# robotic-vision-lab/Learning-Implicitly-From-Spatial-Transformers-Network

Measured on AMD Instinct MI355X. Metric: SDF query-points/sec (B=8, N=20k, 224^2), higher is better.
Workload: dtype fp16

## Files before the change

learning-implicitly-from-spatial-transformers-network_amd/csrc/fused_fc0_kernels.hip:

```cpp
#include "list_common.h"
#include "mfma_common.h"
#include "point_math.h"
#include "gather_math.h"

namespace list {

constexpr int kFusedLds = 163840;
constexpr int kFW = 65536, kFA = 16384;
constexpr int kFAOff = 2 * kFW;


__device__ __forceinline__ int fswz(int row) { return (row >> 1) & 7; }

struct RowProj { int64_t base; int dx, dy; float w00, w01, w10, w11; int valid; };
struct RowProjRec { int64_t base; int dx, dy; float w00, w01, w10, w11; int valid, pad_[3]; };
constexpr int kFProjRecOff = 81920;

template <int X3, bool PROJ = false>
__global__ __launch_bounds__(512, 2) void k_fc0_fused(FusedFc0Params fp) {
  static_assert(!PROJ || X3 == 0, "the projected form is built for fp16 operands");
  constexpr bool F16 = X3 == 0;
  constexpr int KT = F16 ? 64 : 32;
  using M = MapT<F16 ? 1 : 0>;
  __shared__ __attribute__((aligned(16))) char smem[kFusedLds];
  const GemmParams& p = fp.gp;
  const int tid = threadIdx.x;
  const int lane = tid & 63;
  const int wave = __builtin_amdgcn_readfirstlane(tid >> 6);
  const int wm = wave >> 2, wn = wave & 3;
  const int ntiles = p.M / 128;
  const int m0 = xcd_contiguous_block(blockIdx.x, ntiles) * 128;
  const int nk = p.K / KT;
  const int np = fp.n_produced;
  const int64_t lda = (int64_t)(p.lda ? p.lda : p.K) * (F16 ? 2 : 4), ldw = lda;
  const int gap_at = p.k_gap_at, gap = p.k_gap;
  auto ktb = [&](int t) { return (t + (t >= gap_at ? gap : 0)) * 128; };

  const int pc = tid & 7, pr = tid >> 3;
  RowProj rp[2];
  if (np > 0 || PROJ) {
#pragma unroll
    for (int h = 0; h < 2; ++h) {
      const Pt pt = load_point(fp.g, m0 + pr + 64 * h);
      const Proj q = project(fp.trans_mat + pt.b * 12, pt.x, pt.y, pt.z, fp.ms, fp.Ct, fp.clamp_hi);
      rp[h].base = (int64_t)pt.b * fp.ms * fp.ms * fp.Ct + q.o00 + pc * M::V;
      rp[h].dx = q.o01 - q.o00; rp[h].dy = q.o10 - q.o00;
      rp[h].w00 = q.w00; rp[h].w01 = q.w01; rp[h].w10 = q.w10; rp[h].w11 = q.w11;
      rp[h].valid = (pt.valid ? 1 : 0) | (q.dead << 1);
    }
  }
  typename M::Raw taps[2][4];
  auto load_taps = [&](int t) {
#pragma unroll
    for (int h = 0; h < 2; ++h) {
      const int64_t o = rp[h].base + t * KT;
      taps[h][0] = M::load(fp.img_map, o);
      taps[h][1] = M::load(fp.img_map, o + rp[h].dx);
      taps[h][2] = M::load(fp.img_map, o + rp[h].dy);
      taps[h][3] = M::load(fp.img_map, o + rp[h].dy + rp[h].dx);
    }
  };
  auto produce = [&](char* astage) {
#pragma unroll
// ... 120 lines not shown
    if (t + 1 < np) {
      wait_vmcnt<8>();
      produce(smem + kFAOff + nxt * kFA);
      if (t + 2 < np) load_taps(t + 2);
    }
  }

  {
    float* tile = (float*)smem + wave * (32 * kStageLd);
    const int col_in = lane & 15, row_in = 4 * (lane >> 4);
    const int rr = lane >> 3, c8 = (lane & 7) * 8;
    const int64_t row_base = m0 + wm * 64;
    const int col_base = wn * 128;
    bool bad = false;
    __syncthreads();
    const RowProjRec* recs = (const RowProjRec*)(smem + kFProjRecOff);
    if constexpr (PROJ) {
      if (pc == 0) {
#pragma unroll
        for (int h = 0; h < 2; ++h) {
          RowProjRec rc;
          rc.base = rp[h].base; rc.dx = rp[h].dx; rc.dy = rp[h].dy;
          rc.w00 = rp[h].w00; rc.w01 = rp[h].w01; rc.w10 = rp[h].w10; rc.w11 = rp[h].w11; rc.valid = rp[h].valid;
          rc.pad_[0] = rc.pad_[1] = rc.pad_[2] = 0;
          *(RowProjRec*)(smem + kFProjRecOff + (pr + 64 * h) * (int)sizeof(RowProjRec)) = rc;
        }
      }
      __syncthreads();
    }
#pragma unroll
    for (int ih = 0; ih < 2; ++ih)
#pragma unroll
      for (int jh = 0; jh < 2; ++jh) {
        [[maybe_unused]] uint4 ptap[4][4];
        if constexpr (PROJ) {
#pragma unroll
          for (int k = 0; k < 4; ++k) {
            const RowProjRec& rc = recs[wm * 64 + ih * 32 + rr + 8 * k];
            const int64_t o = rc.base + fp.kept + col_base + jh * 64 + c8;
            ptap[k][0] = M::load(fp.img_map, o);
            ptap[k][1] = M::load(fp.img_map, o + rc.dx);
            ptap[k][2] = M::load(fp.img_map, o + rc.dy);
            ptap[k][3] = M::load(fp.img_map, o + rc.dy + rc.dx);
          }
        }
#pragma unroll
        for (int ii = 0; ii < 2; ++ii)
#pragma unroll
          for (int jj = 0; jj < 4; ++jj)
#pragma unroll
            for (int e = 0; e < 4; ++e)
              tile[(ii * 16 + row_in + e) * kStageLd + jj * 16 + col_in] = acc[2 * ih + ii][4 * jh + jj][e];
        __syncthreads();
        const int cb = col_base + jh * 64 + c8;
        const float4 b0 = *(const float4*)(p.bias + cb), b1 = *(const float4*)(p.bias + cb + 4);
        const float bb[8] = {b0.x, b0.y, b0.z, b0.w, b1.x, b1.y, b1.z, b1.w};
#pragma unroll
        for (int k = 0; k < 4; ++k) {
          const int r = rr + 8 * k;
          const float4 x = *(const float4*)(tile + r * kStageLd + c8);
          const float4 y = *(const float4*)(tile + r * kStageLd + c8 + 4);
          const float v[8] = {x.x, x.y, x.z, x.w, y.x, y.y, y.z, y.w};
          float o[8];
          if constexpr (PROJ) {
            const RowProjRec& rc = recs[wm * 64 + ih * 32 + r];
            const float wt[4] = {rc.w00, rc.w01, rc.w10, rc.w11};
            float sm[8];
#pragma unroll
            for (int e = 0; e < 8; ++e) sm[e] = 0.f;
#pragma unroll
            for (int tp = 0; tp < 4; ++tp) {
              float f[8];
              M::unpack(ptap[k][tp], f);
              const bool dead = (rc.valid >> (1 + tp)) & 1;
#pragma unroll
              for (int e = 0; e < 8; ++e) sm[e] = fmaf(dead ? 0.f : f[e], wt[tp], sm[e]);
            }
            const bool live = (rc.valid & 1) != 0;
#pragma unroll
            for (int e = 0; e < 8; ++e) { o[e] = relu_nan((v[e] + (live ? sm[e] : 0.f)) + bb[e]); bad = bad || (o[e] != o[e]); }
          } else {
#pragma unroll
            for (int e = 0; e < 8; ++e) { o[e] = relu_nan(v[e] + bb[e]); bad = bad || (o[e] != o[e]); }
          }
          store8_planes<F16 ? 1 : 0>(p.out_hi, F16 ? nullptr : p.out_lo, (row_base + ih * 32 + r) * p.ldo + cb, o);
        }
        __syncthreads();
      }
    if (p.nan_tiles && __builtin_amdgcn_ballot_w64(bad) != 0 && lane == 0) p.nan_tiles[m0 / 256] = 1;
  }
}

bool fused_fc0_eligible(const GemmParams& gp, int img_f16, int img_C) {
  if (gp.N != 512 || gp.M <= 0 || gp.M % 128 || gp.K % 64 || img_C < 0 || img_C % 64 || img_C > gp.K || !gp.bias ||
      gp.rowvec || gp.a_rows || gp.tile_gate) return false;
  if (gp.lda != gp.ldw || (gp.k_gap && !gp.lda)) return false;
  return gp.fmt == FMT_FP16 ? (img_f16 != 0 && !gp.x3i) : (img_f16 == 0 && gp.x3i != 0);
}

hipError_t launch_fc0_fused(const FusedFc0Params& fp, int terms, hipStream_t s) {
  const dim3 grid(fp.gp.M / 128);
  if (fp.proj) {
    if (fp.gp.fmt != FMT_FP16 || fp.gp.N != 512) return hipErrorInvalidValue;
    hipLaunchKernelGGL((k_fc0_fused<0, true>), grid, dim3(512), 0, s, fp);
  } else if (fp.gp.fmt == FMT_FP16) hipLaunchKernelGGL((k_fc0_fused<0, false>), grid, dim3(512), 0, s, fp);
  else if (terms == 3) hipLaunchKernelGGL((k_fc0_fused<3, false>), grid, dim3(512), 0, s, fp);
  else hipLaunchKernelGGL((k_fc0_fused<1, false>), grid, dim3(512), 0, s, fp);
  return hipGetLastError();
}

}
```

learning-implicitly-from-spatial-transformers-network_amd/csrc/gather_kernels.hip:

```cpp
#include <string.h>

#include "list_common.h"
#include "point_math.h"
#include "gather_math.h"

namespace list {

template <int V>
__device__ __forceinline__ bool any_nan(const float (&a)[V]) {
  bool bad = false;
#pragma unroll
  for (int c = 0; c < V; ++c) bad = bad || (a[c] != a[c]);
  return bad;
}
__device__ __forceinline__ bool wave_any(bool x) { return __builtin_amdgcn_ballot_w64(x) != 0; }
__device__ __forceinline__ void launder(float& x) { asm volatile("" : "+v"(x)); }
__device__ __forceinline__ void launder(int& x) { asm volatile("" : "+v"(x)); }
__device__ __forceinline__ void launder(unsigned& x) { asm volatile("" : "+v"(x)); }
__device__ __forceinline__ void launder(float4& r) { launder(r.x); launder(r.y); launder(r.z); launder(r.w); }
__device__ __forceinline__ void launder(uint4& r) { launder(r.x); launder(r.y); launder(r.z); launder(r.w); }

template <typename M>
__device__ __forceinline__ void tap_fma_masked(typename M::Raw r, float w, bool dead, float (&a)[M::V]) {
  float f[M::V];
// ... 460 lines not shown
      p.z = q[(int64_t)g.perm2 * g.q_sc] * g.scale;
      if (p.valid) row = g.row_of[pt];
    } else {
      p = load_point(g, row);
    }
    ImgPoint ip;
    ip.pr = project(trans_mat + p.b * 12, p.x, p.y, p.z, ms, Ct, clamp_hi);
    ip.row = row; ip.b = p.b; ip.valid = p.valid ? 1 : 0;
    ipt[threadIdx.x] = ip;
  }
  __syncthreads();
  unsigned short* __restrict__ xh = g.x_hi;
  unsigned short* __restrict__ xl = g.x_lo;
  const int64_t img_stride = (int64_t)ms * ms * Ct;
  constexpr int NP = 2;
  const int lq = Ct / M::V;
  const int ppp = lq >= 256 ? 1 : 256 / lq;
  const int span = ppp * NP;
#pragma unroll 1
  for (int i = 0; i < kGatherRows; i += span) {
    for (int u = threadIdx.x; u < ppp * lq; u += 256) {
      const int pp = u / lq, q = u - pp * lq;
      Raw v[NP][4];
#pragma unroll
      for (int k = 0; k < NP; ++k) {
        const int pi = min(i + k * ppp + pp, kGatherRows - 1);
        const ImgPoint& a = ipt[pi];
        const int64_t bo = a.b * img_stride + q * M::V;
        v[k][0] = M::load(img_map, bo + a.pr.o00); v[k][1] = M::load(img_map, bo + a.pr.o01);
        v[k][2] = M::load(img_map, bo + a.pr.o10); v[k][3] = M::load(img_map, bo + a.pr.o11);
      }
// ... 4 lines not shown
        const ImgPoint& a = ipt[pi];
        float r[M::V];
        if constexpr (OUT32) {
          if (q * M::V >= kept) {
            reduce_proj_exact<M>(v[k], a.pr, r);
            float* dst = g.rowvec + (int64_t)a.row * g.rv_stride + (q * M::V - kept);
#pragma unroll
            for (int h = 0; h < M::V / 4; ++h)
              *(float4*)(dst + 4 * h) = a.valid ? make_float4(r[4 * h], r[4 * h + 1], r[4 * h + 2], r[4 * h + 3])
                                                : make_float4(0.f, 0.f, 0.f, 0.f);
            continue;
          }
        }
        tap_mul<M>(v[k][0], a.pr.w00, r); tap_fma<M>(v[k][1], a.pr.w01, r);
        tap_fma<M>(v[k][2], a.pr.w10, r); tap_fma<M>(v[k][3], a.pr.w11, r);
        store_feats<FMT, M::V, true>(xh, xl, (int64_t)a.row * g.Kp + col_off + q * M::V, r, a.valid != 0);
      }
    }
  }
}

template <int FMT>
__global__ __launch_bounds__(256) void k_copy_percep(GatherParams g, const float* __restrict__ pf,
                                                     int64_t sb, int64_t sc, int64_t sn, int Ct,
                                                     int col_off) {
  const int row = blockIdx.x * 256 + threadIdx.x;
  if (row >= g.rows) return;
  const bool valid = row < g.n_valid;
  const int64_t gp = g.p_begin + (valid ? (g.order ? g.order[row] : row) : 0);
  const int b = (int)(gp / g.N);
  const int n = (int)(gp - (int64_t)b * g.N);
// ... 241 lines not shown
      case 64: return launch_vox_level<64, FMT>(g, lv, L.vox_off[l], s, order, rd);
      case 128: return launch_vox_level<128, FMT>(g, lv, L.vox_off[l], s, order, rd);
      case 256: return launch_vox_level<256, FMT>(g, lv, L.vox_off[l], s, order, rd);
      default: return hipErrorInvalidValue;
    }
  };
  auto img = [&]() -> hipError_t {
    if (skip_img) return hipSuccess;
    if (a.percep_proj) {
      if (FMT == FMT_FP16)
        LIST_LAUNCH((k_gather_img<FMT, 1, 1>), dim3(g.rows / kGatherRows), dim3(256), 0, s, order, g, a.percep_proj,
                    a.trans_mat, a.map_size, a.H1, a.clamp_hi, 0, 0);
      else
        LIST_LAUNCH((k_gather_img<FMT, 0, 1>), dim3(g.rows / kGatherRows), dim3(256), 0, s, order, g, a.percep_proj,
                    a.trans_mat, a.map_size, a.H1, a.clamp_hi, 0, 0);
    } else if (a.img_proj) {
      if (FMT == FMT_FP16)
        LIST_LAUNCH((k_gather_img<FMT, 1, 1>), dim3(g.rows / kGatherRows), dim3(256), 0, s, order, g, a.img_map,
                    a.trans_mat, a.map_size, a.img_kept_C + a.H1, a.clamp_hi, L.img_off, a.img_kept_C);
      else
        LIST_LAUNCH((k_gather_img<FMT, 0, 1>), dim3(g.rows / kGatherRows), dim3(256), 0, s, order, g, a.img_map,
                    a.trans_mat, a.map_size, a.img_kept_C + a.H1, a.clamp_hi, L.img_off, a.img_kept_C);
    } else if (a.percep_feat) {
      LIST_LAUNCH(k_copy_percep<FMT>, dim3((g.rows + 255) / 256), dim3(256), 0, s, order, g,
                  a.percep_feat, a.pf_sb, a.pf_sc, a.pf_sn, L.img_C, L.img_off);
    } else if (a.img_dtype == LIST_MAP_F16) {
      LIST_LAUNCH((k_gather_img<FMT, 1>), dim3(g.rows / kGatherRows), dim3(256), 0, s, order, g, a.img_map,
                  a.trans_mat, a.map_size, L.img_C, a.clamp_hi, L.img_off, 0);
    } else {
      LIST_LAUNCH((k_gather_img<FMT, 0>), dim3(g.rows / kGatherRows), dim3(256), 0, s, order, g, a.img_map,
// ... 116 lines not shown
```

learning-implicitly-from-spatial-transformers-network_amd/csrc/gemm_kernels.hip:

```cpp
#include <type_traits>

#include "list_common.h"
#include "mfma_common.h"

namespace list {

constexpr int BM = 256, BN = 256;
constexpr int kLdsBytes = 131072;

template <int TERMS> struct Pipe {
  static constexpr int kPlanes = TERMS == 3 ? 4 : 2;
  static constexpr int BK = TERMS == 3 ? 32 : 64;
  static constexpr int kRowBytes = BK * 2;
  static constexpr int kPlaneBytes = BM * kRowBytes;
  static constexpr int kStageBytes = kPlanes * kPlaneBytes;
  static constexpr int kStages = kLdsBytes / kStageBytes;
  static constexpr int kAhead = kStages - 1;
  static constexpr int kRowsPerPiece = 1024 / kRowBytes;
  static constexpr int kPiecesPerWave = BM / kRowsPerPiece / 8;
  static constexpr int kLoadsPerStage = kPiecesPerWave * kPlanes;
  static constexpr int kWOff = (TERMS == 3 ? 2 : 1) * kPlaneBytes;
  __device__ static __forceinline__ int swz(int row) {
    return kRowBytes == 64 ? ((row >> 2) & 3) : ((row >> 1) & 7);
  }
// ... 339 lines not shown
          store8_planes<FP16>(p.out_hi, p.out_lo, (row_base + c * 32 + r) * p.ldo + col_base + c8, o);
        }
        __syncthreads();
      }
    } else
    staged_epilogue16(acc, smem, wave, lane, [&](int r, int c8, const float (&v)[8]) {
      float o[8];
      const float4 b0 = p.bias ? *(const float4*)(p.bias + col_base + c8) : make_float4(0.f, 0.f, 0.f, 0.f);
      const float4 b1 = p.bias ? *(const float4*)(p.bias + col_base + c8 + 4) : make_float4(0.f, 0.f, 0.f, 0.f);
      const float bb[8] = {b0.x, b0.y, b0.z, b0.w, b1.x, b1.y, b1.z, b1.w};
#pragma unroll
      for (int e = 0; e < 8; ++e) { o[e] = relu_nan(v[e] + bb[e]); bad = bad || (o[e] != o[e]); }
      store8_planes<FP16>(p.out_hi, p.out_lo, (row_base + r) * p.ldo + col_base + c8, o);
    });
    if (p.nan_tiles && __builtin_amdgcn_ballot_w64(bad) != 0 && lane == 0) p.nan_tiles[m0 / BM] = 1;
  } else if (EPI == EPI_MASK_SPLIT) {
    const int64_t row_base = m0 + wm * 128;
    const int col_base = n0 + wn * 64;
    staged_epilogue16(acc, smem, wave, lane, [&](int r, int c8, const float (&v)[8]) {
      const int64_t row = row_base + r;
      const uint4 mk = *(const uint4*)(p.mask + row * p.ldmask + col_base + c8);
      const unsigned mw[4] = {mk.x, mk.y, mk.z, mk.w};
      float o[8];
#pragma unroll
      for (int e = 0; e < 4; ++e) {
        o[2 * e] = (mw[e] & 0x7fffu) ? v[2 * e] : 0.f;
        o[2 * e + 1] = (mw[e] & 0x7fff0000u) ? v[2 * e + 1] : 0.f;
      }
      store8_planes<FP16>(p.out_hi, p.out_lo, row * p.ldo + col_base + c8, o);
    });
// ... 84 lines not shown
    }
  }
}

__device__ __forceinline__ int a_quarter_row(int q, int half) { return (q >> 3) * 128 + half * 64 + (q & 7) * 8; }
__device__ __forceinline__ int w_quarter_row(int q, int half) { return (q >> 2) * 64 + half * 32 + (q & 3) * 8; }

constexpr int kLead = 4;
constexpr int kPpMinK = 512;

template <int EPI, int FP16, bool S16, int X3 = 0>
__global__ __launch_bounds__(512, 2) void k_gemm_nt_pp(GemmParams p) {
  using P = Pipe<1>;
  static_assert(X3 == 0 || (S16 && !FP16), "interleaved split operands: 16x16x32 bf16 only");
  static_assert(P::BK == 64 && P::kRowBytes == 128, "single-plane pipeline");
  __shared__ __attribute__((aligned(16))) char smem[kLdsBytes];
  const int lane = threadIdx.x & 63;
  const int wave = __builtin_amdgcn_readfirstlane(threadIdx.x >> 6);
  const int wm = wave >> 2, wn = wave & 3;
  const int tiles_n = p.N / BN;
  const int ntiles = (p.M / BM) * tiles_n;
  const int tile = xcd_contiguous_block(blockIdx.x, ntiles);
  int m0 = (tile / tiles_n) * BM;
  const int n0 = (tile % tiles_n) * BN;
  if (p.tile_gate && p.tile_gate[tile / tiles_n] == 0) return;
  const char* A = p.a_hi; const char* Wt = p.w_hi;
  int Kk = p.K, lda_e = p.lda ? p.lda : p.K, a_rows_e = p.a_rows ? p.a_rows : p.M;
  [[maybe_unused]] void* dx_out = p.dx;
  if constexpr (EPI == EPI_DX) {
    if (p.n_groups > 0) {
      int mt = tile / tiles_n;
// ... 33 lines not shown
  const int w_row_off = (wn * 64 + frow) * P::kRowBytes;
  const int64_t lda = (int64_t)lda_e * (X3 ? 4 : 2);
  const int64_t ldw = (int64_t)(p.ldw ? p.ldw : p.K) * (X3 ? 4 : 2);
  const int a_last = a_rows_e - 1;
  const int nk = X3 ? Kk / 32 : Kk / P::BK;

  auto stage_quarter = [&](char* sbase, int kbyte, int quarter) {
#pragma unroll
    for (int r = 0; r < 2; ++r) {
      const int q = 2 * wave + r;
      const bool is_a = quarter == 0 || quarter == 3;
      const int row0 = is_a ? a_quarter_row(q, quarter == 3) : w_quarter_row(q, quarter == 2);
      const int row = row0 + lane / 8;
      const int chunk = (lane % 8) ^ P::swz(row);
      const char* g = (is_a ? A + (int64_t)min(m0 + row, a_last) * lda : Wt + (int64_t)(n0 + row) * ldw) + kbyte + chunk * 16;
      if (EPI == EPI_RELU_SPLIT && is_a) glds16_nt(g, sbase + row0 * P::kRowBytes);
      else glds16(g, sbase + (is_a ? 0 : P::kWOff) + row0 * P::kRowBytes);
    }
  };
  auto frag = [&](const char* cur, int plane_off, int row_off, int blk, int ks) -> bf16x8 {
    return *(const bf16x8*)(cur + plane_off + row_off + blk * TR * P::kRowBytes + (((KO * ks + fo) ^ fswz) << 4));
  };

  const int gap_at = p.k_gap_at, gap = p.k_gap;
  auto ktb = [&](int t) { return (t + (t >= gap_at ? gap : 0)) * P::kRowBytes; };
#pragma unroll
  for (int g = 0; g < kLead; ++g)
    if (g / 4 < nk) stage_quarter(smem + ((g / 4) & 1) * P::kStageBytes, ktb(g / 4), g & 3);
  if (nk > 1) wait_vmcnt<2 * (kLead - 4)>(); else wait_vmcnt<0>();
  __builtin_amdgcn_s_barrier();
  if (wm == 1) __builtin_amdgcn_s_barrier();
  const int last_quarter = 4 * nk - 1;

  bf16x8 a[HA][KS], w[2][HW][KS];
  auto k_tile = [&](int t, auto steady) {
    constexpr bool STEADY = decltype(steady)::value;
    const char* cur = smem + (t & 1) * P::kStageBytes;
#pragma unroll
    for (int ph = 0; ph < 4; ++ph) {
      if (ph == 0 || ph == 1) {
#pragma unroll
        for (int ks = 0; ks < KS; ++ks)
#pragma unroll
// ... 314 lines not shown
    hipLaunchKernelGGL((k_gemm_nt<TERMS, EPI, FP16>), dim3(ntiles), dim3(512), 0, s, p);
  }
  return hipGetLastError();
}

template <int TERMS, int FP16>
static hipError_t launch_epi(const GemmParams& p, int epi, hipStream_t s) {
  if (epi == EPI_RELU_SPLIT) return launch_one<TERMS, EPI_RELU_SPLIT, FP16>(p, s);
  if (epi == EPI_F32) return launch_one<TERMS, EPI_F32, FP16>(p, s);
  if (epi == EPI_MASK_SPLIT) return launch_one<TERMS, EPI_MASK_SPLIT, FP16>(p, s);
  if (epi == EPI_DX) return launch_one<TERMS, EPI_DX, FP16>(p, s);
  return launch_one<TERMS, EPI_RELU_DOT, FP16>(p, s);
}

hipError_t launch_gemm(const GemmParams& p, int terms, int epi, hipStream_t s) {
  if (p.n_groups) {
    if (epi != EPI_DX || p.n_groups < 0 || p.n_groups > kGemmMaxGroups) return hipErrorInvalidValue;
    int tiles = 0;
    for (int i = 0; i < p.n_groups; ++i) {
      const GemmGroup& g = p.grp[i];
      if (g.K % 64 || g.K <= 0 || g.m_tiles <= 0 || g.a_rows <= 0 || g.a_rows > g.m_tiles * BM || !g.a || !g.w || !g.out) return hipErrorInvalidValue;
      tiles += g.m_tiles;
    }
    if (tiles * BM != p.M || p.plain_loop) return hipErrorInvalidValue;
  }
  if (p.M % BM || p.N % BN || p.K % 64 || p.M <= 0) return hipErrorInvalidValue;
  if (p.x3i && p.fmt == FMT_FP16) return hipErrorInvalidValue;
  if (epi == EPI_RELU_DOT && p.N != BN) return hipErrorInvalidValue;
  if (p.fmt == FMT_FP16) return launch_epi<1, 1>(p, epi, s);
  if (terms == 3) return launch_epi<3, 0>(p, epi, s);
// ... 5 lines not shown
```

learning-implicitly-from-spatial-transformers-network_amd/csrc/list_capi.hip:

```cpp
#include <string.h>

#include "list_common.h"
#include "list_host.h"

using namespace list;

namespace {

constexpr int64_t kMaxChunkRows = 262144;

bool aligned16(const void* p) { return (reinterpret_cast<uintptr_t>(p) & 15) == 0; }

bool vox_in_place(const ListMap3D& m, ListVoxLevel* lv, int32_t map_dtype) {
  const int64_t C = m.C, W = m.W, H = m.H;
  lv->C = m.C; lv->D = m.D; lv->H = m.H; lv->W = m.W; lv->dtype = LIST_MAP_F32; lv->reserved_ = 0;
  if (m.dtype == LIST_MAP_F16) {
    if (map_dtype != LIST_MAP_F16 || m.C == 1 || (m.C % 8) != 0) return false;
    if (m.sc == 1 && m.sw == C && m.sh == W * C && m.sd == H * W * C && aligned16(m.data) && (m.sb % 8) == 0) {
      lv->data = m.data; lv->image_stride = m.sb; lv->dtype = LIST_MAP_F16; return true;
    }
    return false;
  }
  if (m.C == 1) {
    if (m.sw == 1 && m.sh == W && m.sd == H * W) { lv->data = m.data; lv->image_stride = m.sb; return true; }
// ... 109 lines not shown
  while (fit >= kRowTile && workspace_layout(fit, Kp, H1, H2).total > bytes) fit -= kRowTile;
  return fit >= kRowTile ? fit : 0;
}

int fused_fc0_mode() {
  static const int mode = [] {
    const char* e = getenv("LIST_FUSED_FC0");
    if (!e || !e[0]) return 1;
    if (e[0] == '0' && e[1] == 0) return 0;
    if (e[0] == 'x') return 2;
    if (e[0] == '3' && e[1] == 0) return 3;
    return 1;
  }();
  return mode;
}
bool takes_fused_fc0_any(const ListQueryArgs* a, const FeatLayout& L) {
  if (fused_fc0_mode() == 0) return false;
  if (a->percep_feat || a->percep_proj) return false;
  if (a->img_proj && (a->precision != LIST_PREC_FP16 || fused_fc0_mode() == 2)) return false;
  if ((a->precision == LIST_PREC_FP16) != (a->img_dtype == LIST_MAP_F16)) return false;
  if (a->precision == LIST_PREC_BF16X3 && fused_fc0_mode() != 3) return false;
  if (!a->no_activations || a->no_fused_fc0) return false;
  return a->H1 == 512 && a->img_C > 0 && a->img_C % 64 == 0 && L.img_off == 0 && L.Kp % 64 == 0;
}
int fused_produced_tiles(const ListQueryArgs* a) {
  const int channels = a->img_proj ? a->img_kept_C : a->img_C;
  return fused_fc0_mode() == 2 ? 0 : channels / (a->precision == LIST_PREC_FP16 ? 64 : 32);
}
bool takes_fused_fc0(const ListQueryArgs* a, const FeatLayout& L) {
  return takes_fused_fc0_any(a, L) && fused_fc0_mode() != 2;
}

bool takes_fused_tail(const ListQueryArgs* a) {
  return a->no_activations && a->precision == LIST_PREC_FP16 && a->H2 == 256 && a->H3 == 256 && a->H1 % 64 == 0;
}

}

extern "C" {

const char* list_last_error(void) { return g_err; }
int list_abi_version(void) { return LIST_ABI_VERSION; }

static bool dtype_ok(int32_t d) { return d == LIST_MAP_F32 || d == LIST_MAP_F16; }
static size_t elem_bytes(int32_t d) { return d == LIST_MAP_F16 ? 2 : 4; }
// ... 364 lines not shown
  const int sets = a->stage_events ? (a->stage_event_sets > 0 ? a->stage_event_sets : 1) : 0;
  int chunk = 0;
  for (int64_t p0 = 0; p0 < P; p0 += rows, ++chunk) {
    const int n_valid = (int)((P - p0 < rows) ? (P - p0) : rows);
    const int crow = (n_valid + kRowTile - 1) / kRowTile * kRowTile;
    GatherParams g = make_gather(a, L, ws, p0, n_valid, crow);
    void* const* events = chunk < sets ? a->stage_events + (size_t)chunk * LIST_N_STAGES : nullptr;
    chunk_args.stage_events = events;
    auto mark = [&](int stage) {
      if (events && events[stage]) (void)hipEventRecord((hipEvent_t)events[stage], s);
    };
    mark(LIST_STAGE_BEGIN);
    hipError_t e = hipSuccess;
    if (!a->no_sort) {
      SortBuffers sb;
      const bool want_pix = !takes_fused_fc0(a, L);
      sb.order = (int*)(wsb + ws.order); sb.order_img = want_pix ? (int*)(wsb + ws.order_img) : nullptr;
      sb.row_of = (int*)(wsb + ws.row_of); sb.keys = (int*)(wsb + ws.keys);
      sb.keys2 = (int*)(wsb + ws.keys2); sb.bins = (int*)(wsb + ws.bins);
      e = launch_sort_points(g, *a, sb, s);
      if (e != hipSuccess) return hip_fail(e, "sort launch");
      g.order = sb.order;
      if (want_pix && a->percep_feat == nullptr && a->map_size * ((a->map_size + 3) / 4) <= kSortPixCells) {
        g.order_img = sb.order_img; g.row_of = sb.row_of;
      }
    }
    mark(LIST_STAGE_SORT);
    int* nan_tiles = (int*)(wsb + ws.nan_tiles);
    const bool fused0 = takes_fused_fc0_any(a, L);
    e = launch_gather(g, L, chunk_args, nan_tiles, s, takes_fused_fc0(a, L));
    if (e != hipSuccess) return hip_fail(e, "gather launch");
    mark(LIST_STAGE_TAIL);

    GemmParams gp;
    memset(&gp, 0, sizeof(gp));
    gp.fmt = g.fmt;
    gp.a_hi = wsb + ws.x_hi; gp.a_lo = wsb + ws.x_lo;
    gp.w_hi = wp + pk.w0_hi; gp.w_lo = wp + pk.w0_lo;
    gp.bias = (const float*)(wp + pk.b0);
    gp.M = crow; gp.N = a->H1; gp.K = L.Kp;
    gp.x3i = g.fmt == FMT_FP16 ? 0 : 1;
    if (gp.x3i && (ws.x_lo != ws.x_hi + (size_t)rows * L.Kp * 2 || pk.w0_lo != pk.w0_hi + (size_t)a->H1 * L.Kp * 2))
      return fail(LIST_ERR_ARG, "internal: hi / lo planes of X or of the packed fc_0 weight are not contiguous");
    if (a->percep_proj) {
      const int64_t skip = (int64_t)a->img_C * (gp.x3i ? 4 : 2);
// ... 4 lines not shown
      const int ktile = gp.x3i ? 32 : 64;
      gp.k_gap_at = a->img_kept_C / ktile; gp.k_gap = (a->img_C - a->img_kept_C) / ktile;
      gp.K = L.Kp - (a->img_C - a->img_kept_C); gp.lda = L.Kp; gp.ldw = L.Kp;
      gp.rowvec = (const char*)g.rowvec; gp.rowvec_stride = g.rv_stride * 4;
      if (a->H1 * 4 > L.Kp * 2) return fail(LIST_ERR_UNSUPPORTED, "img_proj: H1 * 4 bytes exceed a row of the feature matrix's lo plane");
    }
    const char* rowvec_of_call = gp.rowvec;
    gp.out_hi = (unsigned short*)(wsb + ws.h1_hi);
    gp.out_lo = terms == 3 ? (unsigned short*)(wsb + ws.h1_lo) : nullptr;
    gp.ldo = a->H1;
    gp.nan_tiles = nan_tiles;
    if (fused0) {
      FusedFc0Params fp;
      fp.gp = gp; fp.g = g; fp.img_map = a->img_map; fp.trans_mat = a->trans_mat;
      fp.ms = a->map_size; fp.Ct = a->img_C; fp.clamp_hi = a->clamp_hi; fp.n_produced = fused_produced_tiles(a);
      fp.proj = 0; fp.kept = 0;
      if (a->img_proj) {
        fp.proj = 1; fp.kept = a->img_kept_C; fp.Ct = a->img_kept_C + a->H1; fp.gp.rowvec = nullptr;
      }
      if (!fused_fc0_eligible(fp.gp, a->img_dtype == LIST_MAP_F16, a->img_proj ? a->img_kept_C : a->img_C))
        return fail(LIST_ERR_ARG, "internal: fused fc_0 taken for arguments it does not support");
      e = launch_fc0_fused(fp, terms, s);
    } else {
      e = launch_gemm(gp, terms, EPI_RELU_SPLIT, s);
    }
    if (e != hipSuccess) return hip_fail(e, "fc_0 launch");
    mark(LIST_STAGE_FC0);
    e = launch_gather_fixup(g, L, chunk_args, nan_tiles, s);
    if (e != hipSuccess) return hip_fail(e, "gather fix-up launch");
    gp.nan_tiles = nullptr; gp.tile_gate = nan_tiles; gp.rowvec = rowvec_of_call;
    e = launch_gemm(gp, terms, EPI_RELU_SPLIT, s);
    if (e != hipSuccess) return hip_fail(e, "gated fc_0 launch");
    gp.tile_gate = nullptr; gp.x3i = 0;
    gp.lda = gp.ldw = 0; gp.rowvec = nullptr; gp.k_gap_at = gp.k_gap = 0;
    mark(LIST_STAGE_EXACT);
    gp.a_hi = wsb + ws.h1_hi; gp.a_lo = wsb + ws.h1_lo;
    gp.w_hi = wp + pk.w1_hi; gp.w_lo = wp + pk.w1_lo;
// ... 39 lines not shown
  if (a->H1 <= 0 || a->H2 <= 0) return fail(LIST_ERR_UNSUPPORTED, "hidden sizes %d/%d/%d", a->H1, a->H2, a->H3);
  const int64_t P = (int64_t)a->B * a->N;
  const int64_t rows = chunk_rows_for(a->workspace_bytes, P, L.Kp, a->H1, a->H2);
  if (rows < kRowTile) return fail(LIST_ERR_WORKSPACE, "workspace of %zu bytes cannot hold one %d-row tile",
                                   a->workspace_bytes, kRowTile);
  plan->rows_per_chunk = rows;
  plan->chunks = (int32_t)((P + rows - 1) / rows);
  plan->fused_tail = takes_fused_tail(a) ? 1 : 0;
  plan->fc0_k = a->percep_proj ? L.Kp - a->img_C : a->img_proj ? L.Kp - (a->img_C - a->img_kept_C) : L.Kp;
  plan->img_proj = a->img_proj ? 1 : 0;
  {
    const Workspace ws = workspace_layout(rows, L.Kp, a->H1, a->H2);
    const int n_valid = (int)(P < rows ? P : rows);
    const GatherParams g = make_gather(a, L, ws, 0, n_valid, (n_valid + kRowTile - 1) / kRowTile * kRowTile);
    plan->box_levels = gather_box_levels(g, L, *a);
    plan->fused_fc0 = takes_fused_fc0(a, L) ? 1 : 0;
  }
  return LIST_OK;
}

int list_gather_features_fwd(const ListQueryArgs* a, float* out, void* stream) {
  FeatLayout L;
  int rc = check_query_common(a, &L);
  if (rc != LIST_OK) return rc;
  if (!out) return fail(LIST_ERR_ARG, "out is NULL");
  if (a->percep_proj || a->img_proj) return fail(LIST_ERR_UNSUPPORTED, "percep_proj / img_proj leave perceptual features out of X");
  const int64_t P = (int64_t)a->B * a->N;
  const int H1 = a->H1 > 0 ? a->H1 : 512, H2 = a->H2 > 0 ? a->H2 : 256;
  const int64_t rows = chunk_rows_for(a->workspace_bytes, P, L.Kp, H1, H2);
  if (rows < kRowTile) return fail(LIST_ERR_WORKSPACE, "workspace too small");
  const Workspace ws = workspace_layout(rows, L.Kp, H1, H2);
// ... 475 lines not shown
```

learning-implicitly-from-spatial-transformers-network_amd/csrc/list_common.h:

```cpp
#pragma once

#include <hip/hip_runtime.h>
#include <hip/hip_ext.h>
#include <stdint.h>
#include <stdlib.h>

#include "list_hip.h"

namespace list {

inline int any_order() {
  static const int flag = [] {
    const char* e = getenv("LIST_LAUNCH_IN_ORDER");
    return (e && e[0] && !(e[0] == '0' && e[1] == 0)) ? 0 : (int)hipExtAnyOrderLaunch;
  }();
  return flag;
}
#define LIST_LAUNCH(kernel, grid, block, lds, s, order, ...) \
  hipExtLaunchKernelGGL(kernel, grid, block, lds, s, nullptr, nullptr, (order), __VA_ARGS__)

template <bool FP16, typename V>
__device__ __forceinline__ void x_store(const V& v, V* p) {
  if (FP16) *p = v;
  else __builtin_nontemporal_store(v, p);
// ... 303 lines not shown
  float* out_f32; int relu;
  const float* w3; const float* b3; float* sdf; int n_valid;
  const int* order;
  int fmt;
  const unsigned short* mask; int ldmask;
  void* dx; int dx_f16; int n_store;
  int plain_loop;
  int* nan_tiles;
  const int* tile_gate;
  int x3i;
  int lda, ldw;
  int a_rows;
  const char* rowvec; int64_t rowvec_stride;
  GemmGroup grp[kGemmMaxGroups]; int n_groups;
  int k_gap_at, k_gap;
};

enum { EPI_RELU_SPLIT = 0, EPI_F32 = 1, EPI_RELU_DOT = 2, EPI_MASK_SPLIT = 3, EPI_DX = 4 };

struct GemmTnParams {
  const char* a_hi; const char* a_lo; int lda;
  const char* b_hi; const char* b_lo; int ldb;
  int M, N, P;
  int splits, steps_per_split;
  float* slab; int ldn;
  int fmt;
  int b_x3i;
};

hipError_t launch_prep_img(const ListMap2D maps[LIST_N_IMG_LEVELS], int B, int map_size, int Ct,
                           int f16, void* out, hipStream_t s, int n_levels = LIST_N_IMG_LEVELS);
hipError_t launch_img_level_rows(const ListMap2D* maps, void* const* outs, int n, int B, int f16, hipStream_t s);
hipError_t launch_proj_resize_sum(const ListMap2D* src, int n_src, int B, int map_size, int Ct, int coff, int f16,
// ... 16 lines not shown
                               hipStream_t s);
bool gather_box_eligible(const GatherParams& g, const ListVoxLevel& lv, int col_off);
hipError_t launch_gather_vox_box(const GatherParams& g, const ListVoxLevel& lv, int col_off, hipStream_t s, int order);
int gather_box_levels(const GatherParams& g, const FeatLayout& L, const ListQueryArgs& a);
hipError_t launch_gather_fixup(const GatherParams& g, const FeatLayout& L, const ListQueryArgs& a,
                               const int* tile_flags, hipStream_t s);
hipError_t launch_percep_pool(const ListPoolArgs& a, hipStream_t s);
hipError_t launch_gemm(const GemmParams& p, int terms, int epi, hipStream_t s);
struct FusedFc0Params {
  GemmParams gp;
  GatherParams g;
  const void* img_map;
  const float* trans_mat;
  int ms, Ct; float clamp_hi;
  int n_produced;
  int proj, kept;
};
bool fused_fc0_eligible(const GemmParams& gp, int img_f16, int img_C);
hipError_t launch_fc0_fused(const FusedFc0Params& fp, int terms, hipStream_t s);
hipError_t launch_mlp_tail(const GemmParams& fc1, const char* w2, const float* b2, const float* w3, const float* b3,
                           float* sdf, const int* order, int n_valid, hipStream_t s);

hipError_t launch_prep_weights_bwd(const ListMlpWeights& w, const FeatLayout& L, const PackedMlpBwd& P,
                                   char* packed, hipStream_t s);
hipError_t launch_gemm_tn(const GemmTnParams& p, int terms, hipStream_t s);
int wgrad_splits(int M, int N, int P, int terms);
hipError_t launch_wgrad_reduce(const float* slab, int splits, int M, int N, int ldn, const FeatLayout* L,
                               const float* scale, float* out, int ldo, hipStream_t s);
hipError_t launch_grad_scale(const float* grad_sdf, int64_t n, int fp16, float* scale, float* db3,
                             float* partial, hipStream_t s);
hipError_t launch_head(const float* grad_sdf, const int* order, int n_valid, int rows, int H3,
// ... 38 lines not shown
```

learning-implicitly-from-spatial-transformers-network_amd/csrc/point_math.h:

```cpp
#pragma once

#include "list_common.h"

namespace list {

struct Pt { float x, y, z; int b; bool valid; };

__device__ __forceinline__ Pt load_point(const GatherParams& g, int row) {
  Pt p;
  p.valid = row < g.n_valid;
  const int64_t gp = g.p_begin + (p.valid ? (g.order ? g.order[row] : row) : 0);
  p.b = (int)(gp / g.N);
  const int n = (int)(gp - (int64_t)p.b * g.N);
  const float* q = g.query + (int64_t)p.b * g.q_sb + (int64_t)n * g.q_sn;
  p.x = q[(int64_t)g.perm0 * g.q_sc] * g.scale;
  p.y = q[(int64_t)g.perm1 * g.q_sc] * g.scale;
  p.z = q[(int64_t)g.perm2 * g.q_sc] * g.scale;
  return p;
}

struct Axis { int i0; int has1; float w0, w1; };
__device__ __forceinline__ Axis axis_setup(float c, int size) {
  float v = ((c + 1.f) * 0.5f) * (float)(size - 1);
  v = (v != v) ? (float)(size - 1) : fminf((float)(size - 1), fmaxf(v, 0.f));
// ... 60 lines not shown
  Proj r;
  const bool x1_out = !(fx + 1.f <= (float)(ms - 1)), y1_out = !(fy + 1.f <= (float)(ms - 1));
  const bool x0_out = !(fx >= 0.f && fx <= (float)(ms - 1)), y0_out = !(fy >= 0.f && fy <= (float)(ms - 1));
  r.dead = ((x0_out || y0_out) ? 1 : 0) | ((x1_out || y0_out) ? 2 : 0) | ((x0_out || y1_out) ? 4 : 0) |
           ((x1_out || y1_out) ? 8 : 0);
  r.o00 = (y0 * ms + x0) * Ct; r.o01 = (y0 * ms + x1) * Ct;
  r.o10 = (y1 * ms + x0) * Ct; r.o11 = (y1 * ms + x1) * Ct;
  r.w00 = wx0 * wy0; r.w01 = wx1 * wy0; r.w10 = wx0 * wy1; r.w11 = wx1 * wy1;
  if ((r.dead & 1) && r.w00 == r.w00) r.w00 = 0.f;
  if ((r.dead & 2) && r.w01 == r.w01) r.w01 = 0.f;
  if ((r.dead & 4) && r.w10 == r.w10) r.w10 = 0.f;
  if ((r.dead & 8) && r.w11 == r.w11) r.w11 = 0.f;
  return r;
}

}
```

Baseline: 84.62 million.

## Move projected image sampling into main GEMM epilogue instead of fused fc0 kernel

For the img_proj fp16 path, the projected sampling of the precomputed fc0 contribution is taken out of the 128-row fused fc0 kernel and placed in a new EPI_RELU_SAMPLE epilogue of the 256x256 GEMM. Per-row projection records are computed during the GEMM prologue and staged in extra LDS. The kept image channels are now gathered separately into the feature buffer with non-accumulating stores, and the k_gap handling is removed from the fused kernel. The intent is to use the more efficient large-tile GEMM for this case. The cost is more LDS per block and an extra gather pass for the kept channels.

```diff
diff --git a/learning-implicitly-from-spatial-transformers-network_amd/csrc/fused_fc0_kernels.hip b/learning-implicitly-from-spatial-transformers-network_amd/csrc/fused_fc0_kernels.hip
--- a/learning-implicitly-from-spatial-transformers-network_amd/csrc/fused_fc0_kernels.hip
+++ b/learning-implicitly-from-spatial-transformers-network_amd/csrc/fused_fc0_kernels.hip
@@ -12,13 +12,8 @@
 
 __device__ __forceinline__ int fswz(int row) { return (row >> 1) & 7; }
 
-struct RowProj { int64_t base; int dx, dy; float w00, w01, w10, w11; int valid; };
-struct RowProjRec { int64_t base; int dx, dy; float w00, w01, w10, w11; int valid, pad_[3]; };
-constexpr int kFProjRecOff = 81920;
-
-template <int X3, bool PROJ = false>
+template <int X3>
 __global__ __launch_bounds__(512, 2) void k_fc0_fused(FusedFc0Params fp) {
-  static_assert(!PROJ || X3 == 0, "the projected form is built for fp16 operands");
   constexpr bool F16 = X3 == 0;
   constexpr int KT = F16 ? 64 : 32;
   using M = MapT<F16 ? 1 : 0>;
@@ -33,20 +28,15 @@
   const int nk = p.K / KT;
   const int np = fp.n_produced;
   const int64_t lda = (int64_t)(p.lda ? p.lda : p.K) * (F16 ? 2 : 4), ldw = lda;
-  const int gap_at = p.k_gap_at, gap = p.k_gap;
-  auto ktb = [&](int t) { return (t + (t >= gap_at ? gap : 0)) * 128; };
+  auto ktb = [&](int t) { return t * 128; };
 
   const int pc = tid & 7, pr = tid >> 3;
-  RowProj rp[2];
-  if (np > 0 || PROJ) {
+  RowProjRec rp[2];
+  if (np > 0) {
 #pragma unroll
     for (int h = 0; h < 2; ++h) {
-      const Pt pt = load_point(fp.g, m0 + pr + 64 * h);
-      const Proj q = project(fp.trans_mat + pt.b * 12, pt.x, pt.y, pt.z, fp.ms, fp.Ct, fp.clamp_hi);
-      rp[h].base = (int64_t)pt.b * fp.ms * fp.ms * fp.Ct + q.o00 + pc * M::V;
-      rp[h].dx = q.o01 - q.o00; rp[h].dy = q.o10 - q.o00;
-      rp[h].w00 = q.w00; rp[h].w01 = q.w01; rp[h].w10 = q.w10; rp[h].w11 = q.w11;
-      rp[h].valid = (pt.valid ? 1 : 0) | (q.dead << 1);
+      rp[h] = row_proj_rec(fp.g, fp.trans_mat, fp.ms, fp.Ct, fp.clamp_hi, m0 + pr + 64 * h);
+      rp[h].base += pc * M::V;
     }
   }
   typename M::Raw taps[2][4];
@@ -197,36 +187,10 @@
     const int col_base = wn * 128;
     bool bad = false;
     __syncthreads();
-    const RowProjRec* recs = (const RowProjRec*)(smem + kFProjRecOff);
-    if constexpr (PROJ) {
-      if (pc == 0) {
-#pragma unroll
-        for (int h = 0; h < 2; ++h) {
-          RowProjRec rc;
-          rc.base = rp[h].base; rc.dx = rp[h].dx; rc.dy = rp[h].dy;
-          rc.w00 = rp[h].w00; rc.w01 = rp[h].w01; rc.w10 = rp[h].w10; rc.w11 = rp[h].w11; rc.valid = rp[h].valid;
-          rc.pad_[0] = rc.pad_[1] = rc.pad_[2] = 0;
-          *(RowProjRec*)(smem + kFProjRecOff + (pr + 64 * h) * (int)sizeof(RowProjRec)) = rc;
-        }
-      }
-      __syncthreads();
-    }
 #pragma unroll
     for (int ih = 0; ih < 2; ++ih)
 #pragma unroll
       for (int jh = 0; jh < 2; ++jh) {
-        [[maybe_unused]] uint4 ptap[4][4];
-        if constexpr (PROJ) {
-#pragma unroll
-          for (int k = 0; k < 4; ++k) {
-            const RowProjRec& rc = recs[wm * 64 + ih * 32 + rr + 8 * k];
-            const int64_t o = rc.base + fp.kept + col_base + jh * 64 + c8;
-            ptap[k][0] = M::load(fp.img_map, o);
-            ptap[k][1] = M::load(fp.img_map, o + rc.dx);
-            ptap[k][2] = M::load(fp.img_map, o + rc.dy);
-            ptap[k][3] = M::load(fp.img_map, o + rc.dy + rc.dx);
-          }
-        }
 #pragma unroll
         for (int ii = 0; ii < 2; ++ii)
 #pragma unroll
@@ -245,27 +209,8 @@
           const float4 y = *(const float4*)(tile + r * kStageLd + c8 + 4);
           const float v[8] = {x.x, x.y, x.z, x.w, y.x, y.y, y.z, y.w};
           float o[8];
-          if constexpr (PROJ) {
-            const RowProjRec& rc = recs[wm * 64 + ih * 32 + r];
-            const float wt[4] = {rc.w00, rc.w01, rc.w10, rc.w11};
-            float sm[8];
-#pragma unroll
-            for (int e = 0; e < 8; ++e) sm[e] = 0.f;
-#pragma unroll
-            for (int tp = 0; tp < 4; ++tp) {
-              float f[8];
-              M::unpack(ptap[k][tp], f);
-              const bool dead = (rc.valid >> (1 + tp)) & 1;
-#pragma unroll
-              for (int e = 0; e < 8; ++e) sm[e] = fmaf(dead ? 0.f : f[e], wt[tp], sm[e]);
-            }
-            const bool live = (rc.valid & 1) != 0;
-#pragma unroll
-            for (int e = 0; e < 8; ++e) { o[e] = relu_nan((v[e] + (live ? sm[e] : 0.f)) + bb[e]); bad = bad || (o[e] != o[e]); }
-          } else {
-#pragma unroll
-            for (int e = 0; e < 8; ++e) { o[e] = relu_nan(v[e] + bb[e]); bad = bad || (o[e] != o[e]); }
-          }
+#pragma unroll
+          for (int e = 0; e < 8; ++e) { o[e] = relu_nan(v[e] + bb[e]); bad = bad || (o[e] != o[e]); }
           store8_planes<F16 ? 1 : 0>(p.out_hi, F16 ? nullptr : p.out_lo, (row_base + ih * 32 + r) * p.ldo + cb, o);
         }
         __syncthreads();
@@ -276,19 +221,16 @@
 
 bool fused_fc0_eligible(const GemmParams& gp, int img_f16, int img_C) {
   if (gp.N != 512 || gp.M <= 0 || gp.M % 128 || gp.K % 64 || img_C < 0 || img_C % 64 || img_C > gp.K || !gp.bias ||
-      gp.rowvec || gp.a_rows || gp.tile_gate) return false;
-  if (gp.lda != gp.ldw || (gp.k_gap && !gp.lda)) return false;
+      gp.rowvec || gp.a_rows || gp.tile_gate || gp.k_gap) return false;
+  if (gp.lda != gp.ldw) return false;
   return gp.fmt == FMT_FP16 ? (img_f16 != 0 && !gp.x3i) : (img_f16 == 0 && gp.x3i != 0);
 }
 
 hipError_t launch_fc0_fused(const FusedFc0Params& fp, int terms, hipStream_t s) {
   const dim3 grid(fp.gp.M / 128);
-  if (fp.proj) {
-    if (fp.gp.fmt != FMT_FP16 || fp.gp.N != 512) return hipErrorInvalidValue;
-    hipLaunchKernelGGL((k_fc0_fused<0, true>), grid, dim3(512), 0, s, fp);
-  } else if (fp.gp.fmt == FMT_FP16) hipLaunchKernelGGL((k_fc0_fused<0, false>), grid, dim3(512), 0, s, fp);
-  else if (terms == 3) hipLaunchKernelGGL((k_fc0_fused<3, false>), grid, dim3(512), 0, s, fp);
-  else hipLaunchKernelGGL((k_fc0_fused<1, false>), grid, dim3(512), 0, s, fp);
+  if (fp.gp.fmt == FMT_FP16) hipLaunchKernelGGL((k_fc0_fused<0>), grid, dim3(512), 0, s, fp);
+  else if (terms == 3) hipLaunchKernelGGL((k_fc0_fused<3>), grid, dim3(512), 0, s, fp);
+  else hipLaunchKernelGGL((k_fc0_fused<1>), grid, dim3(512), 0, s, fp);
   return hipGetLastError();
 }
 
diff --git a/learning-implicitly-from-spatial-transformers-network_amd/csrc/gather_kernels.hip b/learning-implicitly-from-spatial-transformers-network_amd/csrc/gather_kernels.hip
--- a/learning-implicitly-from-spatial-transformers-network_amd/csrc/gather_kernels.hip
+++ b/learning-implicitly-from-spatial-transformers-network_amd/csrc/gather_kernels.hip
@@ -498,7 +498,7 @@
   unsigned short* __restrict__ xl = g.x_lo;
   const int64_t img_stride = (int64_t)ms * ms * Ct;
   constexpr int NP = 2;
-  const int lq = Ct / M::V;
+  const int lq = ((!OUT32 && kept > 0) ? kept : Ct) / M::V;
   const int ppp = lq >= 256 ? 1 : 256 / lq;
   const int span = ppp * NP;
 #pragma unroll 1
@@ -533,7 +533,8 @@
         }
         tap_mul<M>(v[k][0], a.pr.w00, r); tap_fma<M>(v[k][1], a.pr.w01, r);
         tap_fma<M>(v[k][2], a.pr.w10, r); tap_fma<M>(v[k][3], a.pr.w11, r);
-        store_feats<FMT, M::V, true>(xh, xl, (int64_t)a.row * g.Kp + col_off + q * M::V, r, a.valid != 0);
+        if (!OUT32 && kept > 0) store_feats<FMT, M::V, false>(xh, xl, (int64_t)a.row * g.Kp + col_off + q * M::V, r, a.valid != 0);
+        else store_feats<FMT, M::V, true>(xh, xl, (int64_t)a.row * g.Kp + col_off + q * M::V, r, a.valid != 0);
       }
     }
   }
@@ -805,6 +806,11 @@
       else
         LIST_LAUNCH((k_gather_img<FMT, 0, 1>), dim3(g.rows / kGatherRows), dim3(256), 0, s, order, g, a.percep_proj,
                     a.trans_mat, a.map_size, a.H1, a.clamp_hi, 0, 0);
+    } else if (a.img_proj && !g.rowvec) {
+      if (FMT != FMT_FP16 || g.order_img) return hipErrorInvalidValue;
+      if (a.img_kept_C == 0) return hipSuccess;
+      LIST_LAUNCH((k_gather_img<FMT_FP16, 1>), dim3(g.rows / kGatherRows), dim3(256), 0, s, order, g, a.img_map,
+                  a.trans_mat, a.map_size, a.img_kept_C + a.H1, a.clamp_hi, L.img_off, a.img_kept_C);
     } else if (a.img_proj) {
       if (FMT == FMT_FP16)
         LIST_LAUNCH((k_gather_img<FMT, 1, 1>), dim3(g.rows / kGatherRows), dim3(256), 0, s, order, g, a.img_map,
diff --git a/learning-implicitly-from-spatial-transformers-network_amd/csrc/gemm_kernels.hip b/learning-implicitly-from-spatial-transformers-network_amd/csrc/gemm_kernels.hip
--- a/learning-implicitly-from-spatial-transformers-network_amd/csrc/gemm_kernels.hip
+++ b/learning-implicitly-from-spatial-transformers-network_amd/csrc/gemm_kernels.hip
@@ -2,11 +2,14 @@
 
 #include "list_common.h"
 #include "mfma_common.h"
+#include "point_math.h"
+#include "gather_math.h"
 
 namespace list {
 
 constexpr int BM = 256, BN = 256;
 constexpr int kLdsBytes = 131072;
+constexpr int kProjRecBytes = BM * (int)sizeof(RowProjRec);
 
 template <int TERMS> struct Pipe {
   static constexpr int kPlanes = TERMS == 3 ? 4 : 2;
@@ -377,6 +380,65 @@
       store8_planes<FP16>(p.out_hi, p.out_lo, (row_base + r) * p.ldo + col_base + c8, o);
     });
     if (p.nan_tiles && __builtin_amdgcn_ballot_w64(bad) != 0 && lane == 0) p.nan_tiles[m0 / BM] = 1;
+  } else if constexpr (EPI == EPI_RELU_SAMPLE) {
+    using M = MapT<1>;
+    const int64_t row_base = m0 + wm * 128;
+    const int col_base = n0 + wn * 64;
+    float* tile = (float*)smem + wave * (32 * kStageLd);
+    const int rr = lane >> 3, c8 = (lane & 7) * 8;
+    const RowProjRec* recs = (const RowProjRec*)(smem + kLdsBytes) + wm * 128;
+    const float4 b0 = *(const float4*)(p.bias + col_base + c8), b1 = *(const float4*)(p.bias + col_base + c8 + 4);
+    const float bb[8] = {b0.x, b0.y, b0.z, b0.w, b1.x, b1.y, b1.z, b1.w};
+    bool bad = false;
+    __syncthreads();
+#pragma unroll
+    for (int c = 0; c < 4; ++c) {
+      uint4 ptap[4][4];
+#pragma unroll
+      for (int k = 0; k < 4; ++k) {
+        const RowProjRec& rc = recs[c * 32 + rr + 8 * k];
+        const int64_t o = rc.base + p.smp_coff + col_base + c8;
+        ptap[k][0] = M::load(p.smp_map, o);
+        ptap[k][1] = M::load(p.smp_map, o + rc.dx);
+        ptap[k][2] = M::load(p.smp_map, o + rc.dy);
+        ptap[k][3] = M::load(p.smp_map, o + rc.dy + rc.dx);
+      }
+#pragma unroll
+      for (int ii = 0; ii < 2; ++ii)
+#pragma unroll
+        for (int j = 0; j < 4; ++j)
+#pragma unroll
+          for (int e = 0; e < 4; ++e)
+            tile[(ii * 16 + row_in + e) * kStageLd + j * 16 + col_in] = acc[2 * c + ii][j][e];
+      __syncthreads();
+#pragma unroll
+      for (int k = 0; k < 4; ++k) {
+        const int r = rr + 8 * k;
+        const float4 x = *(const float4*)(tile + r * kStageLd + c8);
+        const float4 y = *(const float4*)(tile + r * kStageLd + c8 + 4);
+        const float v[8] = {x.x, x.y, x.z, x.w, y.x, y.y, y.z, y.w};
+        const RowProjRec& rc = recs[c * 32 + r];
+        const float wt[4] = {rc.w00, rc.w01, rc.w10, rc.w11};
+        float sm[8];
+#pragma unroll
+        for (int e = 0; e < 8; ++e) sm[e] = 0.f;
+#pragma unroll
+        for (int tp = 0; tp < 4; ++tp) {
+          float f[8];
+          M::unpack(ptap[k][tp], f);
+          const bool dead = (rc.valid >> (1 + tp)) & 1;
+#pragma unroll
+          for (int e = 0; e < 8; ++e) sm[e] = fmaf(dead ? 0.f : f[e], wt[tp], sm[e]);
+        }
+        const bool live = (rc.valid & 1) != 0;
+        float o[8];
+#pragma unroll
+        for (int e = 0; e < 8; ++e) { o[e] = relu_nan((v[e] + (live ? sm[e] : 0.f)) + bb[e]); bad = bad || (o[e] != o[e]); }
+        store8_planes<FP16>(p.out_hi, p.out_lo, (row_base + c * 32 + r) * p.ldo + col_base + c8, o);
+      }
+      __syncthreads();
+    }
+    if (p.nan_tiles && __builtin_amdgcn_ballot_w64(bad) != 0 && lane == 0) p.nan_tiles[m0 / BM] = 1;
   } else if (EPI == EPI_MASK_SPLIT) {
     const int64_t row_base = m0 + wm * 128;
     const int col_base = n0 + wn * 64;
@@ -491,7 +553,8 @@
   using P = Pipe<1>;
   static_assert(X3 == 0 || (S16 && !FP16), "interleaved split operands: 16x16x32 bf16 only");
   static_assert(P::BK == 64 && P::kRowBytes == 128, "single-plane pipeline");
-  __shared__ __attribute__((aligned(16))) char smem[kLdsBytes];
+  static_assert(EPI != EPI_RELU_SAMPLE || (S16 && FP16 && X3 == 0), "the sampling epilogue: fp16 on the 16x16x32 shape");
+  __shared__ __attribute__((aligned(16))) char smem[kLdsBytes + (EPI == EPI_RELU_SAMPLE ? kProjRecBytes : 0)];
   const int lane = threadIdx.x & 63;
   const int wave = __builtin_amdgcn_readfirstlane(threadIdx.x >> 6);
   const int wm = wave >> 2, wn = wave & 3;
@@ -555,7 +618,7 @@
       const int row = row0 + lane / 8;
       const int chunk = (lane % 8) ^ P::swz(row);
       const char* g = (is_a ? A + (int64_t)min(m0 + row, a_last) * lda : Wt + (int64_t)(n0 + row) * ldw) + kbyte + chunk * 16;
-      if (EPI == EPI_RELU_SPLIT && is_a) glds16_nt(g, sbase + row0 * P::kRowBytes);
+      if ((EPI == EPI_RELU_SPLIT || EPI == EPI_RELU_SAMPLE) && is_a) glds16_nt(g, sbase + row0 * P::kRowBytes);
       else glds16(g, sbase + (is_a ? 0 : P::kWOff) + row0 * P::kRowBytes);
     }
   };
@@ -568,6 +631,11 @@
 #pragma unroll
   for (int g = 0; g < kLead; ++g)
     if (g / 4 < nk) stage_quarter(smem + ((g / 4) & 1) * P::kStageBytes, ktb(g / 4), g & 3);
+  if constexpr (EPI == EPI_RELU_SAMPLE) {
+    if (wm == 0)
+      *((RowProjRec*)(smem + kLdsBytes) + threadIdx.x) =
+          row_proj_rec(p.smp_pts, p.smp_trans_mat, p.smp_ms, p.smp_Ct, p.smp_clamp_hi, m0 + (int)threadIdx.x);
+  }
   if (nk > 1) wait_vmcnt<2 * (kLead - 4)>(); else wait_vmcnt<0>();
   __builtin_amdgcn_s_barrier();
   if (wm == 1) __builtin_amdgcn_s_barrier();
@@ -912,6 +980,14 @@
 }
 
 hipError_t launch_gemm(const GemmParams& p, int terms, int epi, hipStream_t s) {
+  if (epi == EPI_RELU_SAMPLE) {
+    if (p.fmt != FMT_FP16 || p.x3i || p.n_groups || p.rowvec || p.plain_loop || !p.bias || !p.smp_map || !p.smp_trans_mat ||
+        !p.smp_pts.query || p.smp_ms < 2 || p.smp_coff < 0 || p.smp_coff % 8 || p.smp_Ct % 8 || p.smp_coff + p.N > p.smp_Ct ||
+        p.M % BM || p.N % BN || p.K % 64 || p.M <= 0 || p.K <= 0)
+      return hipErrorInvalidValue;
+    hipLaunchKernelGGL((k_gemm_nt_pp<EPI_RELU_SAMPLE, 1, true>), dim3((p.M / BM) * (p.N / BN)), dim3(512), 0, s, p);
+    return hipGetLastError();
+  }
   if (p.n_groups) {
     if (epi != EPI_DX || p.n_groups < 0 || p.n_groups > kGemmMaxGroups) return hipErrorInvalidValue;
     int tiles = 0;
diff --git a/learning-implicitly-from-spatial-transformers-network_amd/csrc/list_capi.hip b/learning-implicitly-from-spatial-transformers-network_amd/csrc/list_capi.hip
--- a/learning-implicitly-from-spatial-transformers-network_amd/csrc/list_capi.hip
+++ b/learning-implicitly-from-spatial-transformers-network_amd/csrc/list_capi.hip
@@ -147,21 +147,28 @@
   }();
   return mode;
 }
-bool takes_fused_fc0_any(const ListQueryArgs* a, const FeatLayout& L) {
+bool runs_fc0_fused_kernel(const ListQueryArgs* a, const FeatLayout& L) {
   if (fused_fc0_mode() == 0) return false;
   if (a->percep_feat || a->percep_proj) return false;
-  if (a->img_proj && (a->precision != LIST_PREC_FP16 || fused_fc0_mode() == 2)) return false;
+  if (a->img_proj) return false;
   if ((a->precision == LIST_PREC_FP16) != (a->img_dtype == LIST_MAP_F16)) return false;
   if (a->precision == LIST_PREC_BF16X3 && fused_fc0_mode() != 3) return false;
   if (!a->no_activations || a->no_fused_fc0) return false;
   return a->H1 == 512 && a->img_C > 0 && a->img_C % 64 == 0 && L.img_off == 0 && L.Kp % 64 == 0;
 }
 int fused_produced_tiles(const ListQueryArgs* a) {
-  const int channels = a->img_proj ? a->img_kept_C : a->img_C;
-  return fused_fc0_mode() == 2 ? 0 : channels / (a->precision == LIST_PREC_FP16 ? 64 : 32);
-}
-bool takes_fused_fc0(const ListQueryArgs* a, const FeatLayout& L) {
-  return takes_fused_fc0_any(a, L) && fused_fc0_mode() != 2;
+  return fused_fc0_mode() == 2 ? 0 : a->img_C / (a->precision == LIST_PREC_FP16 ? 64 : 32);
+}
+bool skips_img_gather(const ListQueryArgs* a, const FeatLayout& L) {
+  return runs_fc0_fused_kernel(a, L) && fused_fc0_mode() != 2;
+}
+bool runs_fc0_sampled(const ListQueryArgs* a, const FeatLayout& L) {
+  if (!a->img_proj || a->precision != LIST_PREC_FP16 || a->img_dtype != LIST_MAP_F16) return false;
+  if (fused_fc0_mode() == 0 || fused_fc0_mode() == 2 || !a->no_activations || a->no_fused_fc0) return false;
+  return a->H1 == 512 && a->img_C % 64 == 0 && L.img_off == 0 && L.Kp % 64 == 0;
+}
+bool fc0_samples_map(const ListQueryArgs* a, const FeatLayout& L) {
+  return skips_img_gather(a, L) || runs_fc0_sampled(a, L);
 }
 
 bool takes_fused_tail(const ListQueryArgs* a) {
@@ -556,7 +563,7 @@
     hipError_t e = hipSuccess;
     if (!a->no_sort) {
       SortBuffers sb;
-      const bool want_pix = !takes_fused_fc0(a, L);
+      const bool want_pix = !fc0_samples_map(a, L);
       sb.order = (int*)(wsb + ws.order); sb.order_img = want_pix ? (int*)(wsb + ws.order_img) : nullptr;
       sb.row_of = (int*)(wsb + ws.row_of); sb.keys = (int*)(wsb + ws.keys);
       sb.keys2 = (int*)(wsb + ws.keys2); sb.bins = (int*)(wsb + ws.bins);
@@ -569,8 +576,13 @@
     }
     mark(LIST_STAGE_SORT);
     int* nan_tiles = (int*)(wsb + ws.nan_tiles);
-    const bool fused0 = takes_fused_fc0_any(a, L);
-    e = launch_gather(g, L, chunk_args, nan_tiles, s, takes_fused_fc0(a, L));
+    const bool fused0 = runs_fc0_fused_kernel(a, L);
+    const bool sampled0 = runs_fc0_sampled(a, L);
+    {
+      GatherParams gg = g;
+      if (sampled0) gg.rowvec = nullptr;
+      e = launch_gather(gg, L, chunk_args, nan_tiles, s, skips_img_gather(a, L));
+    }
     if (e != hipSuccess) return hip_fail(e, "gather launch");
     mark(LIST_STAGE_TAIL);
 
@@ -605,13 +617,15 @@
       FusedFc0Params fp;
       fp.gp = gp; fp.g = g; fp.img_map = a->img_map; fp.trans_mat = a->trans_mat;
       fp.ms = a->map_size; fp.Ct = a->img_C; fp.clamp_hi = a->clamp_hi; fp.n_produced = fused_produced_tiles(a);
-      fp.proj = 0; fp.kept = 0;
-      if (a->img_proj) {
-        fp.proj = 1; fp.kept = a->img_kept_C; fp.Ct = a->img_kept_C + a->H1; fp.gp.rowvec = nullptr;
-      }
-      if (!fused_fc0_eligible(fp.gp, a->img_dtype == LIST_MAP_F16, a->img_proj ? a->img_kept_C : a->img_C))
+      if (!fused_fc0_eligible(fp.gp, a->img_dtype == LIST_MAP_F16, a->img_C))
         return fail(LIST_ERR_ARG, "internal: fused fc_0 taken for arguments it does not support");
       e = launch_fc0_fused(fp, terms, s);
+    } else if (sampled0) {
+      GemmParams sp = gp;
+      sp.rowvec = nullptr; sp.rowvec_stride = 0;
+      sp.smp_map = a->img_map; sp.smp_trans_mat = a->trans_mat; sp.smp_ms = a->map_size;
+      sp.smp_Ct = a->img_kept_C + a->H1; sp.smp_coff = a->img_kept_C; sp.smp_clamp_hi = a->clamp_hi; sp.smp_pts = g;
+      e = launch_gemm(sp, terms, EPI_RELU_SAMPLE, s);
     } else {
       e = launch_gemm(gp, terms, EPI_RELU_SPLIT, s);
     }
@@ -681,7 +695,7 @@
     const int n_valid = (int)(P < rows ? P : rows);
     const GatherParams g = make_gather(a, L, ws, 0, n_valid, (n_valid + kRowTile - 1) / kRowTile * kRowTile);
     plan->box_levels = gather_box_levels(g, L, *a);
-    plan->fused_fc0 = takes_fused_fc0(a, L) ? 1 : 0;
+    plan->fused_fc0 = fc0_samples_map(a, L) ? 1 : 0;
   }
   return LIST_OK;
 }
diff --git a/learning-implicitly-from-spatial-transformers-network_amd/csrc/list_common.h b/learning-implicitly-from-spatial-transformers-network_amd/csrc/list_common.h
--- a/learning-implicitly-from-spatial-transformers-network_amd/csrc/list_common.h
+++ b/learning-implicitly-from-spatial-transformers-network_amd/csrc/list_common.h
@@ -341,9 +341,13 @@
   const char* rowvec; int64_t rowvec_stride;
   GemmGroup grp[kGemmMaxGroups]; int n_groups;
   int k_gap_at, k_gap;
-};
-
-enum { EPI_RELU_SPLIT = 0, EPI_F32 = 1, EPI_RELU_DOT = 2, EPI_MASK_SPLIT = 3, EPI_DX = 4 };
+  const void* smp_map;
+  const float* smp_trans_mat;
+  int smp_ms, smp_Ct, smp_coff; float smp_clamp_hi;
+  GatherParams smp_pts;
+};
+
+enum { EPI_RELU_SPLIT = 0, EPI_F32 = 1, EPI_RELU_DOT = 2, EPI_MASK_SPLIT = 3, EPI_DX = 4, EPI_RELU_SAMPLE = 5 };
 
 struct GemmTnParams {
   const char* a_hi; const char* a_lo; int lda;
@@ -390,7 +394,6 @@
   const float* trans_mat;
   int ms, Ct; float clamp_hi;
   int n_produced;
-  int proj, kept;
 };
 bool fused_fc0_eligible(const GemmParams& gp, int img_f16, int img_C);
 hipError_t launch_fc0_fused(const FusedFc0Params& fp, int terms, hipStream_t s);
diff --git a/learning-implicitly-from-spatial-transformers-network_amd/csrc/point_math.h b/learning-implicitly-from-spatial-transformers-network_amd/csrc/point_math.h
--- a/learning-implicitly-from-spatial-transformers-network_amd/csrc/point_math.h
+++ b/learning-implicitly-from-spatial-transformers-network_amd/csrc/point_math.h
@@ -98,4 +98,19 @@
   return r;
 }
 
+struct RowProjRec { int64_t base; int dx, dy; float w00, w01, w10, w11; int valid, pad_[3]; };
+
+__device__ __forceinline__ RowProjRec row_proj_rec(const GatherParams& g, const float* __restrict__ trans_mat, int ms,
+                                                   int Ct, float clamp_hi, int row) {
+  const Pt pt = load_point(g, row);
+  const Proj q = project(trans_mat + pt.b * 12, pt.x, pt.y, pt.z, ms, Ct, clamp_hi);
+  RowProjRec r;
+  r.base = (int64_t)pt.b * ms * ms * Ct + q.o00;
+  r.dx = q.o01 - q.o00; r.dy = q.o10 - q.o00;
+  r.w00 = q.w00; r.w01 = q.w01; r.w10 = q.w10; r.w11 = q.w11;
+  r.valid = (pt.valid ? 1 : 0) | (q.dead << 1);
+  r.pad_[0] = r.pad_[1] = r.pad_[2] = 0;
+  return r;
 }
+
+}
```

New measurement: 88.60 million, median of 6. 4.7% higher.
